# apache/incubator-predictionio

Hardware: NVIDIA H100
Metric: ALS iterations/sec (higher is better)
Workload: dtype f32

## Files before the change

### incubator-predictionio_b200/csrc/als_pair_kernel.cuh

```cuda
#pragma once
#include <cuda_fp16.h>
#include <cuda_runtime.h>
#include <stdint.h>

#include "als_kernels.cuh"
#include "als_lockstep.cuh"

namespace pio {
namespace pr {

constexpr int KP = 64;
constexpr int CH = 8;
constexpr int RSTR = KP;
constexpr int NSTAGE = 4;
constexpr int STAGE = CH * RSTR;
constexpr int NTILE = 20;
using LL = LsLayout<KP>;
constexpr int SLOT_STRIDE = LL::STRIDE;
constexpr int VSTR = 80;
constexpr int PART_FLOATS = LL::SIZE + KP;
static_assert(NSTAGE * STAGE <= SLOT_STRIDE, "the staging ring lives in the second slot");
static_assert(NSTAGE % 2 == 0, "a loop step consumes two stages");
constexpr int W_BVEC = 2 * SLOT_STRIDE;
constexpr int W_COL = W_BVEC + 2 * VSTR;
constexpr int W_MVAL = W_COL + 2 * VSTR;
constexpr int W_FLOATS = W_MVAL + NSTAGE * CH + 8;
constexpr size_t smem_bytes(int warps) { return sizeof(float) * (size_t)W_FLOATS * warps; }

__device__ __forceinline__ int split_exponent(float vmax) {
  if (!(vmax > 0.f)) return 0;
  if (isinf(vmax)) return -63;
  int x;
  frexpf(vmax, &x);
  const int e = 15 - x;
  return e < -63 ? -63 : e > 63 ? 63 : e;
}
__device__ __forceinline__ float pow2f(int e) { return __int_as_float((127 + e) << 23); }

__global__ void __launch_bounds__(256) abs_max_kernel(const float* __restrict__ x, long long n, unsigned* out) {
  float m = 0.f;
  const long long stride = (long long)gridDim.x * blockDim.x;
  const long long i0 = (long long)blockIdx.x * blockDim.x + threadIdx.x;
  long long tail = 0;
  if ((reinterpret_cast<uintptr_t>(x) & 15) == 0) {
    const long long n4 = n >> 2;
    for (long long i = i0; i < n4; i += stride) {
      const float4 v = __ldg(reinterpret_cast<const float4*>(x) + i);
      m = fmaxf(m, fmaxf(fmaxf(fabsf(v.x), fabsf(v.y)), fmaxf(fabsf(v.z), fabsf(v.w))));
    }
    tail = 4 * n4;
  }
  for (long long i = tail + i0; i < n; i += stride) m = fmaxf(m, fabsf(__ldg(x + i)));
#pragma unroll
  for (int o = 16; o > 0; o >>= 1) m = fmaxf(m, __shfl_xor_sync(0xffffffffu, m, o));
  if ((threadIdx.x & 31) == 0) atomicMax(out, __float_as_uint(m));
}

__device__ __forceinline__ uint64_t pack2(uint32_t x, uint32_t y) {
  uint64_t r;
  asm("mov.b64 %0, {%1, %2};" : "=l"(r) : "r"(x), "r"(y));
  return r;
}
__device__ __forceinline__ void mma_f16_p(float (&d)[4], const uint32_t (&a)[4], uint64_t b) {
  asm volatile(
      "{\n .reg .b32 b0, b1;\n mov.b64 {b0, b1}, %8;\n"
      "mma.sync.aligned.m16n8k16.row.col.f32.f16.f16.f32 {%0,%1,%2,%3}, {%4,%5,%6,%7}, {b0,b1}, {%0,%1,%2,%3};\n}\n"
      : "+f"(d[0]), "+f"(d[1]), "+f"(d[2]), "+f"(d[3])
      : "r"(a[0]), "r"(a[1]), "r"(a[2]), "r"(a[3]), "l"(b));
}
__device__ __forceinline__ void mma_f16_zp(float (&d)[4], const uint32_t (&a)[4], uint64_t b) {
  asm volatile(
      "{\n .reg .b32 b0, b1;\n mov.b64 {b0, b1}, %4;\n"
      "mma.sync.aligned.m16n8k16.row.col.f32.f16.f16.f32 {%0,%1,%2,%3}, {%5,%6,%7,%8}, {b0,b1}, {%9,%9,%9,%9};\n}\n"
      : "=f"(d[0]), "=f"(d[1]), "=f"(d[2]), "=f"(d[3])
      : "l"(b), "r"(a[0]), "r"(a[1]), "r"(a[2]), "r"(a[3]), "f"(0.f));
}

__device__ __forceinline__ void split2(float a, float b, uint32_t& hi, uint32_t& lo) {
  const __half2 h = __floats2half2_rn(a, b);
  const float2 hf = __half22float2(h);
  const __half2 l = __floats2half2_rn(__fsub_rn(a, hf.x), __fsub_rn(b, hf.y));
  hi = *reinterpret_cast<const uint32_t*>(&h);
  lo = *reinterpret_cast<const uint32_t*>(&l);
}

template <bool IMPLICIT>
__device__ __forceinline__ void accumulate_row(const SolveParams& p, long long beg, long long end, float s, float unscale,
                                               const float* __restrict__ yty, float* ring, float* mval, float* slot,
                                               float* bv) {
  const int lane = threadIdx.x & 31;
  const int g = lane >> 2, t = lane & 3;
  const int nchunks = 2 * (int)((end - beg + 2 * CH - 1) / (2 * CH));
  const int prow = lane >> 4, psl = lane & 15;

  int nidx;
  float nval;
  auto prefetch_meta = [&](int c) {
    const long long e = beg + (long long)c * CH + (lane & 15);
    nidx = (c < nchunks && e < end) ? __ldg(p.idx + e) : -1;
    nval = (lane < 2 * CH && c < nchunks && e < end) ? __ldg(p.val + e) : 0.f;
  };
  auto issue = [&](int c) {
    if (c < nchunks) {
#pragma unroll
      for (int h = 0; h < 2; ++h) {
        float* sbuf = ring + ((c + h) % NSTAGE) * STAGE;
#pragma unroll
        for (int j = 0; j < 4; ++j) {
          const int r = 2 * j + prow;
          const int src = __shfl_sync(0xffffffffu, nidx, CH * h + r);
          float4* d4 = reinterpret_cast<float4*>(sbuf + r * RSTR + ((psl * 4) ^ (8 * r)));
          if (src >= 0) cp_async16(d4, p.src + (size_t)src * KP + psl * 4);
          else *d4 = make_float4(0.f, 0.f, 0.f, 0.f);
        }
      }
      if (lane < 2 * CH) mval[(c % NSTAGE) * CH + lane] = nval;
    }
    cp_async_commit();
  };

  float acc[NTILE][4];
#pragma unroll
  for (int i = 0; i < NTILE; ++i)
#pragma unroll
    for (int e = 0; e < 4; ++e) acc[i][e] = 0.f;
  float pb[4][2];
#pragma unroll
  for (int i = 0; i < 4; ++i) pb[i][0] = pb[i][1] = 0.f;

  int xo[4];
#pragma unroll
  for (int q = 0; q < 4; ++q) xo[q] = g + 8 * (q ^ t);

  prefetch_meta(0);
  issue(0);
  prefetch_meta(2);

#pragma unroll 1
  for (int c = 0; c < nchunks; c += 2) {
    cp_async_wait<0>();
    __syncwarp();
    issue(c + 2);
    prefetch_meta(c + 4);
    const float* XA = ring + (c % NSTAGE) * STAGE + t * RSTR;
    const float* XB = XA + STAGE;
    const float* mv = mval + (c % NSTAGE) * CH;
    float wb[4], sc[4];
    {
      const float r[4] = {mv[t], mv[t + 4], mv[CH + t], mv[CH + t + 4]};
#pragma unroll
      for (int q = 0; q < 4; ++q) {
        wb[q] = r[q];
        sc[q] = s;
        if (IMPLICIT) {
          const float c1 = p.alpha * fabsf(r[q]);
          sc[q] = __fmul_rn(sqrtf(c1), s);
          wb[q] = r[q] > 0.f ? 1.f + c1 : 0.f;
        }
      }
    }
    uint32_t hi[4][4], lo[4][4];
#pragma unroll
    for (int i = 0; i < 4; ++i) {
#pragma unroll
      for (int e = 0; e < 2; ++e) {
        const int q = 2 * i + e;
        const int c0 = xo[q & 3] + 32 * (q >> 2), c4 = 4 * RSTR + xo[q & 3] + 32 * (1 - (q >> 2));
        const float a0 = XA[c0], a4 = XA[c4], b0 = XB[c0], b4 = XB[c4];
        pb[i][e] = fmaf(wb[0], a0, pb[i][e]);
        pb[i][e] = fmaf(wb[1], a4, pb[i][e]);
        pb[i][e] = fmaf(wb[2], b0, pb[i][e]);
        pb[i][e] = fmaf(wb[3], b4, pb[i][e]);
        split2(__fmul_rn(a0, sc[0]), __fmul_rn(a4, sc[1]), hi[i][e], lo[i][e]);
        split2(__fmul_rn(b0, sc[2]), __fmul_rn(b4, sc[3]), hi[i][e + 2], lo[i][e + 2]);
      }
    }
#pragma unroll
    for (int j = 0; j < 8; ++j) {
      const int bi = j >> 1, be = j & 1;
      const uint64_t bh = pack2(hi[bi][be], hi[bi][be + 2]), bl = pack2(lo[bi][be], lo[bi][be + 2]);
#pragma unroll
      for (int i = bi; i < 4; ++i) {
        const int tile = i * (i + 1) + j;
        float d[4];
        mma_f16_zp(d, lo[i], bh);
        mma_f16_p(d, hi[i], bl);
        mma_f16_p(d, hi[i], bh);
        acc[tile][0] += d[0];
        acc[tile][1] += d[1];
        acc[tile][2] += d[2];
        acc[tile][3] += d[3];
      }
    }
  }
  cp_async_wait<0>();
  __syncwarp();

#pragma unroll
  for (int i = 0; i < 4; ++i)
#pragma unroll
    for (int e = 0; e < 2; ++e) {
      float v = pb[i][e];
      v += __shfl_xor_sync(0xffffffffu, v, 1);
      v += __shfl_xor_sync(0xffffffffu, v, 2);
      if (t == 0) bv[16 * i + 8 * e + g] = v;
    }
  {
    const float* yl = yty ? yty + g * KP + 2 * t : nullptr;
    int tile = 0;
#pragma unroll
    for (int i = 0; i < 4; ++i) {
#pragma unroll
      for (int j = 0; j <= 2 * i + 1; ++j, ++tile) {
        const int cb = j >> 1;
        const int cc = 8 * (j & 1) + 2 * t;
        float d0 = acc[tile][0] * unscale, d1 = acc[tile][1] * unscale;
        float d2 = acc[tile][2] * unscale, d3 = acc[tile][3] * unscale;
        if (yl) {
          const float2 y0 = __ldg(reinterpret_cast<const float2*>(yl + 16 * i * KP + 8 * j));
          const float2 y1 = __ldg(reinterpret_cast<const float2*>(yl + (16 * i + 8) * KP + 8 * j));
          d0 += y0.x; d1 += y0.y;
          d2 += y1.x; d3 += y1.y;
        }
        if (cb < i) {
          *reinterpret_cast<float2*>(slot + LL::offd(i, cb, g, cc)) = make_float2(d0, d1);
          *reinterpret_cast<float2*>(slot + LL::offd(i, cb, g + 8, cc)) = make_float2(d2, d3);
        } else {
          if (cc <= g) slot[LL::diag(i, g, cc)] = d0;
          if (cc + 1 <= g) slot[LL::diag(i, g, cc + 1)] = d1;
          if (cc <= g + 8) slot[LL::diag(i, g + 8, cc)] = d2;
          if (cc + 1 <= g + 8) slot[LL::diag(i, g + 8, cc + 1)] = d3;
        }
      }
    }
  }
  __syncwarp();
}

__device__ __forceinline__ void fill_identity(float* slot, float* bv) {
  const int lane = threadIdx.x & 31;
  for (int o = lane; o < LL::SIZE; o += 32) slot[o] = 0.f;
  __syncwarp();
  for (int r = lane; r < KP; r += 32) {
    slot[LL::at(r, r)] = 1.f;
    bv[r] = 0.f;
  }
  __syncwarp();
}

template <bool IMPLICIT, int WARPS>
__global__ void __launch_bounds__(32 * WARPS, 12 / WARPS) als_solve_pair_kernel(const SolveParams p, int n_items) {
  extern __shared__ __align__(16) float smem_all[];
  const int warp = threadIdx.x >> 5;
  float* smem = smem_all + warp * W_FLOATS;
  float* slot0 = smem;
  float* slot1 = smem + SLOT_STRIDE;
  float* ring = slot1;
  float* bvec = smem + W_BVEC;
  float* colbuf = smem + W_COL;
  float* mval = smem + W_MVAL;
  const int lane = threadIdx.x & 31;
  const int grp = lane >> 4;
  const int npairs = (n_items + 1) >> 1;
  const float c1_root_max = IMPLICIT ? sqrtf(p.alpha * __uint_as_float(__ldg(p.absmax + 1))) : 1.f;
  const int e = split_exponent(__uint_as_float(__ldg(p.absmax)) * c1_root_max);
  const float s = pow2f(e), unscale = pow2f(-2 * e);

#pragma unroll 1
  for (int base = blockIdx.x * WARPS; base < npairs; base += gridDim.x * WARPS) {
    const int pair = base + warp;
    int row0 = -1, row1 = -1;
    if (pair < npairs) {
#pragma unroll 1
      for (int h = 0; h < 2; ++h) {
        const int item = 2 * pair + h;
        float* slot = h ? slot1 : slot0;
        float* bv = bvec + h * VSTR;
        if (item >= n_items) {
          fill_identity(slot, bv);
          continue;
        }
        long long beg, end;
        if (p.partial) {
          beg = p.wl_beg[item];
          end = p.wl_end[item];
        } else {
          const int r = p.row_begin + item;
          beg = p.ptr[r];
          end = p.ptr[r + 1];
          if (h) row1 = r;
          else row0 = r;
        }
        accumulate_row<IMPLICIT>(p, beg, end, s, unscale, IMPLICIT && !p.partial ? p.yty : nullptr, ring, mval, slot, bv);
        if (p.partial) {
          float* out = p.partial + (size_t)item * PART_FLOATS;
          for (int o = lane; o < LL::SIZE / 4; o += 32)
            reinterpret_cast<float4*>(out)[o] = reinterpret_cast<const float4*>(slot)[o];
          for (int o = lane; o < KP; o += 32) out[LL::SIZE + o] = bv[o];
          __syncwarp();
        }
      }
    }
    if (p.partial) continue;
    if (WARPS > 1) __syncthreads();
    if (pair < npairs) {
      const int myrow = grp ? row1 : row0;
      const int rr = myrow < 0 ? p.row_begin : myrow;
      chol_lockstep<KP>(grp ? slot1 : slot0, bvec + grp * VSTR, p.lambda * p.nreg[rr], p.k, colbuf + grp * VSTR,
                        p.dst + (size_t)(p.dst_row_offset + rr) * KP, myrow >= 0, p.fail);
      __syncwarp();
    }
  }
}

template <bool IMPLICIT>
__global__ void __launch_bounds__(32, 12) als_finish_pair_kernel(const SolveParams p, const int* __restrict__ row_part_ptr,
                                                                  int n_rows) {
  extern __shared__ __align__(16) float smem[];
  float* bvec = smem + W_BVEC;
  float* colbuf = smem + W_COL;
  const int lane = threadIdx.x & 31;
  const int grp = lane >> 4;
  const int npairs = (n_rows + 1) >> 1;
#pragma unroll 1
  for (int pair = blockIdx.x; pair < npairs; pair += gridDim.x) {
#pragma unroll 1
    for (int h = 0; h < 2; ++h) {
      const int r = 2 * pair + h;
      float* slot = smem + h * SLOT_STRIDE;
      float* bv = bvec + h * VSTR;
      if (r >= n_rows) {
        fill_identity(slot, bv);
        continue;
      }
      const int p0 = row_part_ptr[r], p1 = row_part_ptr[r + 1];
      for (int o = lane; o < PART_FLOATS / 4; o += 32) {
        float4 s = make_float4(0.f, 0.f, 0.f, 0.f);
        for (int q = p0; q < p1; ++q) {
          const float4 v = __ldg(reinterpret_cast<const float4*>(p.partial + (size_t)q * PART_FLOATS) + o);
          s.x += v.x; s.y += v.y; s.z += v.z; s.w += v.w;
        }
        if (o < LL::SIZE / 4) reinterpret_cast<float4*>(slot)[o] = s;
        else reinterpret_cast<float4*>(bv)[o - LL::SIZE / 4] = s;
      }
      __syncwarp();
      if (IMPLICIT) {
        ls_add_yty<KP>(slot, p.yty);
        __syncwarp();
      }
    }
    const int myrow = 2 * pair + grp;
    const bool valid = myrow < n_rows;
    const int rr = valid ? myrow : 0;
    chol_lockstep<KP>(smem + grp * SLOT_STRIDE, bvec + grp * VSTR, p.lambda * p.nreg[rr], p.k, colbuf + grp * VSTR,
                      p.dst + (size_t)(p.dst_row_offset + rr) * KP, valid, p.fail);
    __syncwarp();
  }
}

}
}
```

Measured before the change: 35.64.

## Prefetch next row's first gather stage during current row's epilogue

Splits the cp.async staging into reusable helpers and adds a start_next callback so that the first chunk of the next row (the second row of a pair, or the next partial work item) is issued before the current row's reduction and store epilogue runs. This hides the gather latency at row boundaries instead of starting each row with a cold pipeline. The partial path is restructured into a per-warp loop that walks items and writes into slot0 only. This adds control-flow complexity, and relies on the ring stage 0 being free once the last wait has completed.

```diff
diff --git a/incubator-predictionio_b200/csrc/als_pair_kernel.cuh b/incubator-predictionio_b200/csrc/als_pair_kernel.cuh
--- a/incubator-predictionio_b200/csrc/als_pair_kernel.cuh
+++ b/incubator-predictionio_b200/csrc/als_pair_kernel.cuh
@@ -84,40 +84,47 @@
   lo = *reinterpret_cast<const uint32_t*>(&l);
 }
 
-template <bool IMPLICIT>
-__device__ __forceinline__ void accumulate_row(const SolveParams& p, long long beg, long long end, float s, float unscale,
+__device__ __forceinline__ void load_meta(const SolveParams& p, long long e0, long long end, int& nidx, float& nval) {
+  const int lane = threadIdx.x & 31;
+  const long long e = e0 + (lane & 15);
+  nidx = e < end ? __ldg(p.idx + e) : -1;
+  nval = (lane < 2 * CH && e < end) ? __ldg(p.val + e) : 0.f;
+}
+
+__device__ __forceinline__ void stage_step(const SolveParams& p, int nidx, float nval, int stage, float* ring, float* mval) {
+  const int lane = threadIdx.x & 31;
+  const int prow = lane >> 4, psl = lane & 15;
+#pragma unroll
+  for (int h = 0; h < 2; ++h) {
+    float* sbuf = ring + (stage + h) * STAGE;
+#pragma unroll
+    for (int j = 0; j < 4; ++j) {
+      const int r = 2 * j + prow;
+      const int src = __shfl_sync(0xffffffffu, nidx, CH * h + r);
+      float4* d4 = reinterpret_cast<float4*>(sbuf + r * RSTR + ((psl * 4) ^ (8 * r)));
+      if (src >= 0) cp_async16(d4, p.src + (size_t)src * KP + psl * 4);
+      else *d4 = make_float4(0.f, 0.f, 0.f, 0.f);
+    }
+  }
+  if (lane < 2 * CH) mval[stage * CH + lane] = nval;
+}
+
+__device__ __forceinline__ void start_row(const SolveParams& p, long long beg, long long end, float* ring, float* mval,
+                                          int& nidx, float& nval) {
+  load_meta(p, beg, end, nidx, nval);
+  stage_step(p, nidx, nval, 0, ring, mval);
+  cp_async_commit();
+  load_meta(p, beg + 2 * CH, end, nidx, nval);
+}
+
+template <bool IMPLICIT, class StartNext>
+__device__ __forceinline__ void accumulate_row(const SolveParams& p, long long beg, long long end, StartNext start_next,
+                                               int& nidx, float& nval, float s, float unscale,
                                                const float* __restrict__ yty, float* ring, float* mval, float* slot,
                                                float* bv) {
   const int lane = threadIdx.x & 31;
   const int g = lane >> 2, t = lane & 3;
   const int nchunks = 2 * (int)((end - beg + 2 * CH - 1) / (2 * CH));
-  const int prow = lane >> 4, psl = lane & 15;
-
-  int nidx;
-  float nval;
-  auto prefetch_meta = [&](int c) {
-    const long long e = beg + (long long)c * CH + (lane & 15);
-    nidx = (c < nchunks && e < end) ? __ldg(p.idx + e) : -1;
-    nval = (lane < 2 * CH && c < nchunks && e < end) ? __ldg(p.val + e) : 0.f;
-  };
-  auto issue = [&](int c) {
-    if (c < nchunks) {
-#pragma unroll
-      for (int h = 0; h < 2; ++h) {
-        float* sbuf = ring + ((c + h) % NSTAGE) * STAGE;
-#pragma unroll
-        for (int j = 0; j < 4; ++j) {
-          const int r = 2 * j + prow;
-          const int src = __shfl_sync(0xffffffffu, nidx, CH * h + r);
-          float4* d4 = reinterpret_cast<float4*>(sbuf + r * RSTR + ((psl * 4) ^ (8 * r)));
-          if (src >= 0) cp_async16(d4, p.src + (size_t)src * KP + psl * 4);
-          else *d4 = make_float4(0.f, 0.f, 0.f, 0.f);
-        }
-      }
-      if (lane < 2 * CH) mval[(c % NSTAGE) * CH + lane] = nval;
-    }
-    cp_async_commit();
-  };
 
   float acc[NTILE][4];
 #pragma unroll
@@ -131,17 +138,14 @@
   int xo[4];
 #pragma unroll
   for (int q = 0; q < 4; ++q) xo[q] = g + 8 * (q ^ t);
-
-  prefetch_meta(0);
-  issue(0);
-  prefetch_meta(2);
 
 #pragma unroll 1
   for (int c = 0; c < nchunks; c += 2) {
     cp_async_wait<0>();
     __syncwarp();
-    issue(c + 2);
-    prefetch_meta(c + 4);
+    if (c + 2 < nchunks) stage_step(p, nidx, nval, (c + 2) % NSTAGE, ring, mval);
+    cp_async_commit();
+    if (c + 4 < nchunks) load_meta(p, beg + (long long)(c + 4) * CH, end, nidx, nval);
     const float* XA = ring + (c % NSTAGE) * STAGE + t * RSTR;
     const float* XB = XA + STAGE;
     const float* mv = mval + (c % NSTAGE) * CH;
@@ -195,6 +199,7 @@
   }
   cp_async_wait<0>();
   __syncwarp();
+  start_next();
 
 #pragma unroll
   for (int i = 0; i < 4; ++i)
@@ -266,48 +271,63 @@
   const int e = split_exponent(__uint_as_float(__ldg(p.absmax)) * c1_root_max);
   const float s = pow2f(e), unscale = pow2f(-2 * e);
 
-#pragma unroll 1
-  for (int base = blockIdx.x * WARPS; base < npairs; base += gridDim.x * WARPS) {
+  const int stride = gridDim.x * WARPS;
+  int nidx;
+  float nval;
+  if (p.partial) {
+    int item = 2 * (blockIdx.x * WARPS + warp);
+    if (item >= n_items) return;
+    long long beg = p.wl_beg[item], end = p.wl_end[item];
+    start_row(p, beg, end, ring, mval, nidx, nval);
+#pragma unroll 1
+    while (true) {
+      const int next = (item & 1) == 0 && item + 1 < n_items ? item + 1
+                       : 2 * (item / 2 + stride) < n_items  ? 2 * (item / 2 + stride)
+                                                            : -1;
+      auto start_next = [&] {
+        if (next >= 0) start_row(p, __ldg(p.wl_beg + next), __ldg(p.wl_end + next), ring, mval, nidx, nval);
+      };
+      accumulate_row<IMPLICIT>(p, beg, end, start_next, nidx, nval, s, unscale, nullptr, ring, mval, slot0, bvec);
+      float* out = p.partial + (size_t)item * PART_FLOATS;
+      for (int o = lane; o < LL::SIZE / 4; o += 32)
+        reinterpret_cast<float4*>(out)[o] = reinterpret_cast<const float4*>(slot0)[o];
+      for (int o = lane; o < KP; o += 32) out[LL::SIZE + o] = bvec[o];
+      __syncwarp();
+      if (next < 0) return;
+      item = next;
+      beg = __ldg(p.wl_beg + item);
+      end = __ldg(p.wl_end + item);
+    }
+  }
+
+#pragma unroll 1
+  for (int base = blockIdx.x * WARPS; base < npairs; base += stride) {
     const int pair = base + warp;
-    int row0 = -1, row1 = -1;
+    const int r0 = p.row_begin + 2 * pair;
+    const bool two = 2 * pair + 1 < n_items;
+    float ridge = 0.f;
     if (pair < npairs) {
+      start_row(p, __ldg(p.ptr + r0), __ldg(p.ptr + r0 + 1), ring, mval, nidx, nval);
 #pragma unroll 1
       for (int h = 0; h < 2; ++h) {
-        const int item = 2 * pair + h;
-        float* slot = h ? slot1 : slot0;
-        float* bv = bvec + h * VSTR;
-        if (item >= n_items) {
-          fill_identity(slot, bv);
-          continue;
-        }
-        long long beg, end;
-        if (p.partial) {
-          beg = p.wl_beg[item];
-          end = p.wl_end[item];
-        } else {
-          const int r = p.row_begin + item;
-          beg = p.ptr[r];
-          end = p.ptr[r + 1];
-          if (h) row1 = r;
-          else row0 = r;
-        }
-        accumulate_row<IMPLICIT>(p, beg, end, s, unscale, IMPLICIT && !p.partial ? p.yty : nullptr, ring, mval, slot, bv);
-        if (p.partial) {
-          float* out = p.partial + (size_t)item * PART_FLOATS;
-          for (int o = lane; o < LL::SIZE / 4; o += 32)
-            reinterpret_cast<float4*>(out)[o] = reinterpret_cast<const float4*>(slot)[o];
-          for (int o = lane; o < KP; o += 32) out[LL::SIZE + o] = bv[o];
-          __syncwarp();
-        }
-      }
-    }
-    if (p.partial) continue;
+        if (h && !two) {
+          fill_identity(slot1, bvec + VSTR);
+          break;
+        }
+        auto start_next = [&] {
+          if (!h && two) start_row(p, __ldg(p.ptr + r0 + 1), __ldg(p.ptr + r0 + 2), ring, mval, nidx, nval);
+        };
+        accumulate_row<IMPLICIT>(p, __ldg(p.ptr + r0 + h), __ldg(p.ptr + r0 + h + 1), start_next, nidx, nval, s, unscale,
+                                 IMPLICIT ? p.yty : nullptr, ring, mval, h ? slot1 : slot0, bvec + h * VSTR);
+      }
+      if (grp == 0 || two) ridge = p.lambda * p.nreg[r0 + grp];
+    }
     if (WARPS > 1) __syncthreads();
     if (pair < npairs) {
-      const int myrow = grp ? row1 : row0;
-      const int rr = myrow < 0 ? p.row_begin : myrow;
-      chol_lockstep<KP>(grp ? slot1 : slot0, bvec + grp * VSTR, p.lambda * p.nreg[rr], p.k, colbuf + grp * VSTR,
-                        p.dst + (size_t)(p.dst_row_offset + rr) * KP, myrow >= 0, p.fail);
+      const bool valid = grp == 0 || two;
+      const int rr = valid ? r0 + grp : p.row_begin;
+      chol_lockstep<KP>(grp ? slot1 : slot0, bvec + grp * VSTR, ridge, p.k, colbuf + grp * VSTR,
+                        p.dst + (size_t)(p.dst_row_offset + rr) * KP, valid, p.fail);
       __syncwarp();
     }
   }
```

New measurement: 35.79, median of 6. No clear change (+0.4%).
